# Themaister/Granite

Hardware: NVIDIA H100
Metric: frames/sec (higher is better)
Workload: dtype f32

## Files before the change

granite_b200/csrc/grb_post.cu:

```cuda
#include "grb_common.cuh"

#include <cooperative_groups.h>

#include <algorithm>
#include <cstdio>
#include <cstdlib>

namespace grb
{
namespace
{
constexpr int kBlockX = 32;
constexpr int kBlockY = 8;

inline dim3 grid_for(int w, int rows) { return dim3((w + kBlockX - 1) / kBlockX, (rows + kBlockY - 1) / kBlockY, 1); }

template <bool DynamicExposure, typename HdrTexel = uint32_t>
__global__ void __launch_bounds__(kBlockX *kBlockY) bloom_threshold_kernel(View<const HdrTexel> hdr, const float *__restrict__ lum,
                                                                          View<uint2> out, int y0, int y1, float inv_w, float inv_h)
{
	int x = blockIdx.x * kBlockX + threadIdx.x;
	int y = y0 + blockIdx.y * kBlockY + threadIdx.y;
	if (x >= out.w || y >= y1)
		return;
// ... 420 lines not shown
	float3 a0 = sample_unorm8(in, u + dx * k0, v + dy * k0);
	float3 a1 = sample_unorm8(in, u + dx * k1, v + dy * k1);
	float3 rgbA = make_float3(0.5f * (a0.x + a1.x), 0.5f * (a0.y + a1.y), 0.5f * (a0.z + a1.z));
	float3 b0 = sample_unorm8(in, u + dx * -0.5f, v + dy * -0.5f);
	float3 b1 = sample_unorm8(in, u + dx * 0.5f, v + dy * 0.5f);
	float3 rgbB = make_float3(rgbA.x * 0.5f + 0.25f * (b0.x + b1.x), rgbA.y * 0.5f + 0.25f * (b0.y + b1.y), rgbA.z * 0.5f + 0.25f * (b0.z + b1.z));
	float lumaB = luma_of(rgbB);
	float3 c = ((lumaB < lumaMin) || (lumaB > lumaMax)) ? rgbA : rgbB;
	uint32_t px;
	if (SrgbTarget)
		px = linear_to_srgb8(decode_srgb1(c.x)) | (linear_to_srgb8(decode_srgb1(c.y)) << 8) | (linear_to_srgb8(decode_srgb1(c.z)) << 16);
	else
		px = float_to_unorm8(c.x) | (float_to_unorm8(c.y) << 8) | (float_to_unorm8(c.z) << 16);
	out.at(x, y) = px | 0xff000000u;
#undef fetch_unorm8
#undef sample_unorm8
}

__device__ __forceinline__ float3 hdr_to_taa(float3 c)
{
	c = make_float3(c.x * 8.0f, c.y * 8.0f, c.z * 8.0f);
	float r = 1.0f / (fmax_(c.x, fmax_(c.y, c.z)) + 1.0f);
	c = make_float3(c.x * r, c.y * r, c.z * r);
	return make_float3(0.25f * c.x + 0.5f * c.y + 0.25f * c.z, 0.5f * c.y - 0.25f * c.x - 0.25f * c.z, 0.5f * c.x - 0.5f * c.z);
}

__device__ __forceinline__ float3 taa_to_hdr(float3 c)
{
	float tmp = c.x - c.y;
	float3 rgb = make_float3(fclamp(tmp + c.z, 0.0f, 0.999f), fclamp(c.x + c.y, 0.0f, 0.999f), fclamp(tmp - c.z, 0.0f, 0.999f));
	float r = 1.0f / (1.0f - fmax_(rgb.x, fmax_(rgb.y, rgb.z)));
	return make_float3((1.0f / 8.0f) * rgb.x * r, (1.0f / 8.0f) * rgb.y * r, (1.0f / 8.0f) * rgb.z * r);
}

__device__ __forceinline__ float3 min3(float3 a, float3 b) { return make_float3(fmin_(a.x, b.x), fmin_(a.y, b.y), fmin_(a.z, b.z)); }
__device__ __forceinline__ float3 max3(float3 a, float3 b) { return make_float3(fmax_(a.x, b.x), fmax_(a.y, b.y), fmax_(a.z, b.z)); }

template <bool Aabb>
__device__ __forceinline__ float3 clamp_box(float3 color, float3 lo, float3 hi)
{
	if (!Aabb)
		return make_float3(fclamp(color.x, lo.x, hi.x), fclamp(color.y, lo.y, hi.y), fclamp(color.z, lo.z, hi.z));
	float3 center = make_float3(0.5f * (lo.x + hi.x), 0.5f * (lo.y + hi.y), 0.5f * (lo.z + hi.z));
	float3 radius = make_float3(fmax_(0.5f * (hi.x - lo.x), 0.0001f), fmax_(0.5f * (hi.y - lo.y), 0.0001f), fmax_(0.5f * (hi.z - lo.z), 0.0001f));
	float3 v = make_float3(color.x - center.x, color.y - center.y, color.z - center.z);
	float3 units = make_float3(v.x / radius.x, v.y / radius.y, v.z / radius.z);
	float max_unit = fmax_(fmax_(fabsf(units.x), fabsf(units.y)), fabsf(units.z));
	if (max_unit > 1.0f)
		return make_float3(center.x + v.x / max_unit, center.y + v.y / max_unit, center.z + v.z / max_unit);
	return color;
}

template <typename HdrTexel>
struct TaaInputsT
{
	View<const HdrTexel> hdr;
	View<const float> depth;
	View<const uint32_t> mv;
	View<const uint2> history;
};
using TaaInputs = TaaInputsT<uint32_t>;

__device__ __forceinline__ float3 sample_rgb16f(const View<const uint2> &im, float u, float v)
{
	float4 s = sample_rgba16f(im, u, v);
	return make_float3(s.x, s.y, s.z);
}

__device__ __forceinline__ float3 sample_catmull_rom(const View<const uint2> &tex, float u, float v, float4 rt)
{
	float spx = u * rt.z, spy = v * rt.w;
	float t1x = floorf(spx - 0.5f) + 0.5f, t1y = floorf(spy - 0.5f) + 0.5f;
	float fx = spx - t1x, fy = spy - t1y;
#define GRB_W0(f) ((f) * (-0.5f + (f) * (1.0f - 0.5f * (f))))
#define GRB_W1(f) (1.0f + (f) * (f) * (-2.5f + 1.5f * (f)))
#define GRB_W2(f) ((f) * (0.5f + (f) * (2.0f - 1.5f * (f))))
#define GRB_W3(f) ((f) * (f) * (-0.5f + 0.5f * (f)))
	float w0x = GRB_W0(fx), w1x = GRB_W1(fx), w2x = GRB_W2(fx), w3x = GRB_W3(fx);
	float w0y = GRB_W0(fy), w1y = GRB_W1(fy), w2y = GRB_W2(fy), w3y = GRB_W3(fy);
#undef GRB_W0
#undef GRB_W1
#undef GRB_W2
#undef GRB_W3
	float w12x = w1x + w2x, w12y = w1y + w2y;
	float o12x = w2x / (w1x + w2x), o12y = w2y / (w1y + w2y);
	float t0x = (t1x - 1.0f) * rt.x, t0y = (t1y - 1.0f) * rt.y;
	float t3x = (t1x + 2.0f) * rt.x, t3y = (t1y + 2.0f) * rt.y;
	float t12x = (t1x + o12x) * rt.x, t12y = (t1y + o12y) * rt.y;
	float3 result = make_float3(0.0f, 0.0f, 0.0f);
#define GRB_ACC(UU, VV, WA, WB)                      \
	{                                                \
		float4 s4 = sample_rgba16f_snap(tex, (UU), (VV)); float3 s = make_float3(s4.x, s4.y, s4.z); \
		result.x += s.x * (WA) * (WB);               \
		result.y += s.y * (WA) * (WB);               \
		result.z += s.z * (WA) * (WB);               \
	}
	GRB_ACC(t0x, t0y, w0x, w0y)
	GRB_ACC(t12x, t0y, w12x, w0y)
	GRB_ACC(t3x, t0y, w3x, w0y)
	GRB_ACC(t0x, t12y, w0x, w12y)
	GRB_ACC(t12x, t12y, w12x, w12y)
	GRB_ACC(t3x, t12y, w3x, w12y)
	GRB_ACC(t0x, t3y, w0x, w3y)
	GRB_ACC(t12x, t3y, w12x, w3y)
	GRB_ACC(t3x, t3y, w3x, w3y)
#undef GRB_ACC
	return result;
}

struct Mat4
{
	float m[16];
};

template <int Quality, bool History, typename HdrTexel = uint32_t>
__global__ void __launch_bounds__(kBlockX *kBlockY) taa_kernel(TaaInputsT<HdrTexel> in, Mat4 reproj, View<uint32_t> out_color, View<uint2> out_history, int y0,
                                                              int y1, float4 rt)
{
	int x = blockIdx.x * kBlockX + threadIdx.x;
	int y = y0 + blockIdx.y * kBlockY + threadIdx.y;
	if (x >= out_color.w || y >= y1)
		return;
	const int w = in.hdr.w, h = in.hdr.h;
#define GRB_CUR(DX, DY) hdr_to_taa(fetch_hdr_clamped(in.hdr, x + (DX), y + (DY)))
	float3 current = GRB_CUR(0, 0);
	float3 out_c = current;
	if (History)
	{
		float u = ((float)x + 0.5f) * rt.x, v = ((float)y + 0.5f) * rt.y;
		float d;
		uint32_t mvp;
#define GRB_TRY(PX, PY)                                                 \
	{                                                                   \
		int qx = iclamp((PX), 0, w - 1), qy = iclamp((PY), 0, h - 1);   \
		float dd = __ldg(&in.depth.at(qx, qy));                         \
		if (dd > d)                                                     \
		{                                                               \
			d = dd;                                                     \
			mvp = __ldg(&in.mv.at(qx, qy));                             \
		}                                                               \
	}
		if (Quality == 2)
		{
			int qx = iclamp(x + 1, 0, w - 1), qy = iclamp(y + 1, 0, h - 1);
			d = __ldg(&in.depth.at(qx, qy));
			mvp = __ldg(&in.mv.at(qx, qy));
			GRB_TRY(x - 1, y) GRB_TRY(x, y) GRB_TRY(x, y - 1) GRB_TRY(x - 1, y - 1)
			GRB_TRY(x + 1, y) GRB_TRY(x + 1, y - 1)
			GRB_TRY(x - 1, y + 1) GRB_TRY(x, y + 1)
		}
		else
		{
			int qx = iclamp(x - 1, 0, w - 1);
			d = __ldg(&in.depth.at(qx, y));
			mvp = __ldg(&in.mv.at(qx, y));
			GRB_TRY(x, y) GRB_TRY(x, y - 1) GRB_TRY(x, y + 1) GRB_TRY(x + 1, y)
		}
#undef GRB_TRY
		float mvx = h2f((uint16_t)(mvp & 0xffffu)), mvy = h2f((uint16_t)(mvp >> 16));
		float old_u, old_v;
		if (mvx == 0.0f && mvy == 0.0f)
		{
			float cx = 2.0f * u - 1.0f, cy = 2.0f * v - 1.0f;
			const float *m = reproj.m;
			float px = m[0] * cx + m[4] * cy + m[8] * d + m[12] * 1.0f;
			float py = m[1] * cx + m[5] * cy + m[9] * d + m[13] * 1.0f;
			float pw = m[3] * cx + m[7] * cy + m[11] * d + m[15] * 1.0f;
			old_u = px / pw;
			old_v = py / pw;
			mvx = u - old_u;
			mvy = v - old_v;
		}
		else
		{
			old_u = u - mvx;
			old_v = v - mvy;
		}
		float3 hist = Quality == 2 ? sample_catmull_rom(in.history, old_u, old_v, rt) : sample_rgb16f(in.history, old_u, old_v);
		float mv_len = sqrtf(mvx * mvx + mvy * mvy);
		float mv_fast = fmin_(mv_len * 50.0f, 1.0f);
		float gamma = fmix(1.5f, 0.5f, mv_fast);
		hist = make_float3(fclamp(hist.x, 0.0f, 1.0f), fclamp(hist.y, -1.0f, 1.0f), fclamp(hist.z, -1.0f, 1.0f));
		float lerp_factor = (1.0f + 2.0f * mv_fast) / 16.0f;

		float3 c11 = current;
		float3 c01 = GRB_CUR(-1, 0), c21 = GRB_CUR(+1, 0), c10 = GRB_CUR(0, -1), c12 = GRB_CUR(0, +1);
		float3 lo = c11, hi = c11;
		if (Quality == 0 || Quality == 1)
		{
			lo = min3(lo, c01); lo = min3(lo, c21); lo = min3(lo, c10); lo = min3(lo, c12);
			hi = max3(hi, c01); hi = max3(hi, c21); hi = max3(hi, c10); hi = max3(hi, c12);
		}
		if (Quality >= 1)
		{
			float3 corner_lo = lo, corner_hi = hi;
			float3 c00 = GRB_CUR(-1, -1), c22 = GRB_CUR(+1, +1), c02 = GRB_CUR(-1, +1), c20 = GRB_CUR(+1, -1);
			if (Quality == 1)
			{
				lo = min3(lo, c00); lo = min3(lo, c22); lo = min3(lo, c02); lo = min3(lo, c20);
				hi = max3(hi, c00); hi = max3(hi, c22); hi = max3(hi, c02); hi = max3(hi, c20);
				lo = make_float3(0.5f * (corner_lo.x + lo.x), 0.5f * (corner_lo.y + lo.y), 0.5f * (corner_lo.z + lo.z));
				hi = make_float3(0.5f * (corner_hi.x + hi.x), 0.5f * (corner_hi.y + hi.y), 0.5f * (corner_hi.z + hi.z));
			}
			else
			{
#define GRB_M1(C) ((c00.C + 2.0f * c01.C + c02.C + 2.0f * c10.C + 4.0f * c11.C + 2.0f * c12.C + c20.C + 2.0f * c21.C + c22.C) / 16.0f)
#define GRB_M2(C)                                                                                                                            \
	(c00.C * c00.C + 2.0f * c01.C * c01.C + c02.C * c02.C + 2.0f * c10.C * c10.C + 4.0f * c11.C * c11.C + 2.0f * c12.C * c12.C + c20.C * c20.C + \
	 2.0f * c21.C * c21.C + c22.C * c22.C)
				float3 m1 = make_float3(GRB_M1(x), GRB_M1(y), GRB_M1(z));
				float3 m2 = make_float3(GRB_M2(x), GRB_M2(y), GRB_M2(z));
#undef GRB_M1
#undef GRB_M2
				float3 sigma = make_float3(sqrtf(fmax_(m2.x / 16.0f - m1.x * m1.x, 0.0f)), sqrtf(fmax_(m2.y / 16.0f - m1.y * m1.y, 0.0f)),
				                           sqrtf(fmax_(m2.z / 16.0f - m1.z * m1.z, 0.0f)));
				lo = make_float3(m1.x - gamma * sigma.x, m1.y - gamma * sigma.y, m1.z - gamma * sigma.z);
				hi = make_float3(m1.x + gamma * sigma.x, m1.y + gamma * sigma.y, m1.z + gamma * sigma.z);
			}
		}
		hist = clamp_box<Quality != 0>(hist, lo, hi);
		out_c = make_float3(fmix(hist.x, current.x, lerp_factor), fmix(hist.y, current.y, lerp_factor), fmix(hist.z, current.z, lerp_factor));
	}
#undef GRB_CUR
	float3 color = taa_to_hdr(out_c);
	out_color.at(x, y) = pack_r11g11b10(color.x, color.y, color.z);
	out_history.at(x, y) = pack_rgba16f(make_float4(out_c.x, out_c.y, out_c.z, 1.0f));
}

__device__ __forceinline__ float4 sample_rgba16f_cg(const View<const uint2> &im, float u, float v)
{
	Bilin s = bilin_setup(u, v, im.w, im.h);
	float4 t00 = unpack_rgba16f(__ldcg(&im.at(s.x0, s.y0)));
	float4 t10 = unpack_rgba16f(__ldcg(&im.at(s.x1, s.y0)));
	float4 t01 = unpack_rgba16f(__ldcg(&im.at(s.x0, s.y1)));
	float4 t11 = unpack_rgba16f(__ldcg(&im.at(s.x1, s.y1)));
	return bilin_mix4(t00, t10, t01, t11, s.a, s.b);
}

__device__ __forceinline__ float4 tent9_cg(const View<const uint2> &src, float u, float v, float off, float inv_in_w, float inv_in_h)
{
	const float du = off * inv_in_w, dv = off * inv_in_h;
	const float um = u + (-du), up = u + du;
	const float vm = v + (-dv), vp = v + dv;
	float4 s = sample_rgba16f_cg(src, u, v);
	float4 acc = make_float4(0.25f * s.x, 0.25f * s.y, 0.25f * s.z, 0.25f * s.w);
#define GRB_TAP(W, U, V)                     \
	s = sample_rgba16f_cg(src, (U), (V));    \
	acc.x += (W)*s.x;                        \
	acc.y += (W)*s.y;                        \
	acc.z += (W)*s.z;                        \
	acc.w += (W)*s.w;
	GRB_TAP(0.0625f, um, vp)
	GRB_TAP(0.125f, u, vp)
	GRB_TAP(0.0625f, up, vp)
	GRB_TAP(0.125f, um, v)
	GRB_TAP(0.125f, up, v)
	GRB_TAP(0.0625f, um, vm)
	GRB_TAP(0.125f, u, vm)
	GRB_TAP(0.0625f, up, vm)
#undef GRB_TAP
	return acc;
}

struct TailArgs
{
	View<const uint2> d0;
	View<uint2> d1, d2, d3, u2, u1;
	View<const uint2> history;
	float lerp_d3;
	float *lum;
	float lerp_lum, lo, hi;
	View<uint2> u0;
	int u0_y0, u0_y1;
	const uint32_t *wait_flags;
	int wait_count;
	uint32_t wait_epoch;
	uint32_t *error_word;
	unsigned max_spins;
};

constexpr int kTailThreads = 1024;

__device__ __forceinline__ void tail_level(const View<const uint2> &src, const View<uint2> &dst, float off, const View<const uint2> *history, float lerp,
                                          unsigned first_cta, unsigned num_ctas, int y0 = 0, int y1 = -1)
{
	const float inv_w = 1.0f / (float)dst.w, inv_h = 1.0f / (float)dst.h, inv_in_w = 1.0f / (float)src.w, inv_in_h = 1.0f / (float)src.h;
	if (y1 < 0)
		y1 = dst.h;
	const int total = dst.w * (y1 - y0);
	for (int i = (int)((blockIdx.x - first_cta) * kTailThreads + threadIdx.x); i < total; i += (int)(num_ctas * kTailThreads))
	{
		const int yr = i / dst.w, x = i - yr * dst.w, y = y0 + yr;
		const float u = ((float)x + 0.5f) * inv_w, v = ((float)y + 0.5f) * inv_h;
		float4 value = tent9_cg(src, u, v, off, inv_in_w, inv_in_h);
		if (history)
		{
			const float4 hs = unpack_rgba16f(__ldg(&history->at(x, y)));
			value = make_float4(fmix(hs.x, value.x, lerp), fmix(hs.y, value.y, lerp), fmix(hs.z, value.z, lerp), fmix(hs.w, value.w, 1.0f));
		}
		dst.at(x, y) = pack_rgba16f(value);
	}
}

__global__ void __launch_bounds__(kTailThreads) bloom_tail_kernel(const TailArgs a)
{
	namespace cg = cooperative_groups;
	cg::grid_group grid = cg::this_grid();
	__shared__ float s_grid[kLumFastMaxSamples];
	__shared__ float s_part[64];
	auto as_src = [](const View<uint2> &v) { return View<const uint2>{ v.p, v.w, v.h, v.pitch }; };
	if (a.wait_flags)
	{
		if ((int)threadIdx.x < a.wait_count)
			for (unsigned spins = 0; (int32_t)(load_acquire_system(a.wait_flags + threadIdx.x) - a.wait_epoch) < 0; spins++)
			{
				if (spins > a.max_spins)
				{
					if (blockIdx.x == 0)
						printf("granite_b200: timed out waiting for rank %d's band of frame %u\n", (int)threadIdx.x, a.wait_epoch);
					if (a.error_word)
					{
						*reinterpret_cast<volatile uint32_t *>(a.error_word) = (GRB_DEVICE_ERROR_PEER_TIMEOUT << 24) | ((uint32_t)threadIdx.x << 16) | (a.wait_epoch & 0xffffu);
						__threadfence_system();
					}
					break;
				}
				__nanosleep(128);
			}
		__syncthreads();
	}
	tail_level(a.d0, a.d1, 1.75f, nullptr, 0.0f, 0u, gridDim.x);
	grid.sync();
	tail_level(as_src(a.d1), a.d2, 1.75f, nullptr, 0.0f, 0u, gridDim.x);
	grid.sync();
	tail_level(as_src(a.d2), a.d3, 1.75f, a.history.p ? &a.history : nullptr, a.lerp_d3, 0u, gridDim.x);
	grid.sync();
	const bool lum_cta = a.lum != nullptr && blockIdx.x == 0 && gridDim.x > 1;
	if (a.lum != nullptr && (lum_cta || gridDim.x == 1))
	{
		const View<const uint2> d3 = as_src(a.d3);
		const int size_x = d3.w / 2, size_y = d3.h / 2;
		const float inv_sx = 1.0f / (float)size_x, inv_sy = 1.0f / (float)size_y;
		for (int i = threadIdx.x; i < size_x * size_y; i += kTailThreads)
		{
			const int sy = i / size_x, sx = i - sy * size_x;
			s_grid[i] = sample_rgba16f_cg(d3, ((float)sx + 0.5f) * inv_sx, ((float)sy + 0.5f) * inv_sy).w;
		}
		__syncthreads();
		if (threadIdx.x < 64)
		{
			const int iter_y = (size_y + 7) >> 3, iter_x = (size_x + 7) >> 3;
			const int lx = threadIdx.x & 7, ly = threadIdx.x >> 3;
			float total = 0.0f;
			for (int y = 0; y < iter_y; y++)
				for (int x = 0; x < iter_x; x++)
				{
					const int sx = x * 8 + lx, sy = y * 8 + ly;
					if (sx < size_x && sy < size_y)
						total += s_grid[sy * size_x + sx];
				}
			s_part[threadIdx.x] = total;
		}
		luminance_tail(s_part, threadIdx.x, size_x, size_y, inv_sx, inv_sy, a.lum, a.lerp_lum, a.lo, a.hi);
	}
	if (!lum_cta)
		tail_level(as_src(a.d3), a.u2, 0.875f, nullptr, 0.0f, a.lum != nullptr && gridDim.x > 1 ? 1u : 0u, a.lum != nullptr && gridDim.x > 1 ? gridDim.x - 1u : gridDim.x);
	grid.sync();
	tail_level(as_src(a.u2), a.u1, 0.875f, nullptr, 0.0f, 0u, gridDim.x);
	if (a.u0.p)
	{
		grid.sync();
		tail_level(as_src(a.u1), a.u0, 0.875f, nullptr, 0.0f, 0u, gridDim.x, a.u0_y0, a.u0_y1);
	}
}
}
}

namespace grb
{
bool launch_tent_tiled(bool up, const GrbImage *in, const GrbImage *history, float lerp, const GrbImage *out, GrbRows rows, cudaStream_t stream, int32_t *rc);
bool launch_tonemap_fast(const GrbImage *hdr, const GrbImage *bloom, const float *luminance, float exposure, const GrbImage *out, GrbRows rows, cudaStream_t stream,
                         int32_t *rc);
bool launch_fxaa_fast(const GrbImage *in, const GrbImage *out, GrbRows rows, cudaStream_t stream, int32_t *rc);
bool launch_taa_fast(const GrbImage *hdr, const GrbImage *depth, const GrbImage *mv, const GrbImage *history, const float *reproj16, const GrbImage *out_color,
                     const GrbImage *out_history, GrbRows rows, cudaStream_t stream, int32_t *rc);
}

using namespace grb;

extern "C" int32_t grb_bloom_threshold(const GrbImage *hdr, const float *luminance, const GrbImage *out, GrbRows rows, void *stream)
{
	const bool hdr16 = image_ok(hdr, GRB_FORMAT_R16G16B16A16_SFLOAT, 8);
	if ((!hdr16 && !image_ok(hdr, GRB_FORMAT_B10G11R11_UFLOAT_PACK32, 4)) || !image_ok(out, GRB_FORMAT_R16G16B16A16_SFLOAT, 8))
	{
		set_last_error("grb_bloom_threshold: hdr must be B10G11R11_UFLOAT or R16G16B16A16_SFLOAT and out R16G16B16A16_SFLOAT");
		return GRB_ERR_UNSUPPORTED_FORMAT;
	}
	rows = full_rows(rows, out->height);
	if (rows.y1 <= rows.y0)
		return GRB_OK;
	auto o = view_of<uint2>(out);
	dim3 grid = grid_for(out->width, rows.y1 - rows.y0), block(kBlockX, kBlockY);
	float inv_w = 1.0f / (float)out->width, inv_h = 1.0f / (float)out->height;
	if (hdr16)
	{
		if (luminance)
			bloom_threshold_kernel<true, uint2><<<grid, block, 0, as_stream(stream)>>>(view_of<const uint2>(hdr), luminance, o, rows.y0, rows.y1, inv_w, inv_h);
		else
			bloom_threshold_kernel<false, uint2><<<grid, block, 0, as_stream(stream)>>>(view_of<const uint2>(hdr), nullptr, o, rows.y0, rows.y1, inv_w, inv_h);
		return check_launch("grb_bloom_threshold");
	}
	if (luminance)
		bloom_threshold_kernel<true><<<grid, block, 0, as_stream(stream)>>>(view_of<const uint32_t>(hdr), luminance, o, rows.y0, rows.y1, inv_w, inv_h);
	else
		bloom_threshold_kernel<false><<<grid, block, 0, as_stream(stream)>>>(view_of<const uint32_t>(hdr), nullptr, o, rows.y0, rows.y1, inv_w, inv_h);
	return check_launch("grb_bloom_threshold");
}

extern "C" int32_t grb_bloom_downsample(const GrbImage *in, const GrbImage *history, float lerp, const GrbImage *out, GrbRows rows, void *stream)
{
	if (!image_ok(in, GRB_FORMAT_R16G16B16A16_SFLOAT, 8) || !image_ok(out, GRB_FORMAT_R16G16B16A16_SFLOAT, 8) ||
	    (history && (!image_ok(history, GRB_FORMAT_R16G16B16A16_SFLOAT, 8) || history->width != out->width || history->height != out->height)))
	{
		set_last_error("grb_bloom_downsample: images must be R16G16B16A16_SFLOAT and history must match out");
		return GRB_ERR_UNSUPPORTED_FORMAT;
	}
	if (history && history->data == out->data)
	{
		set_last_error("grb_bloom_downsample: history must not alias the output");
		return GRB_ERR_INVALID_ARGUMENT;
	}
	rows = full_rows(rows, out->height);
	if (rows.y1 <= rows.y0)
		return GRB_OK;
	{
		int32_t rc = GRB_OK;
		if (launch_tent_tiled(false, in, history, lerp, out, rows, as_stream(stream), &rc))
			return rc;
	}
	dim3 grid = grid_for(out->width, rows.y1 - rows.y0), block(kBlockX, kBlockY);
	float inv_w = 1.0f / (float)out->width, inv_h = 1.0f / (float)out->height;
	float inv_in_w = 1.0f / (float)in->width, inv_in_h = 1.0f / (float)in->height;
	if (history)
		bloom_downsample_kernel<true><<<grid, block, 0, as_stream(stream)>>>(view_of<const uint2>(in), view_of<const uint2>(history), lerp,
		                                                                      view_of<uint2>(out), rows.y0, rows.y1, inv_w, inv_h, inv_in_w, inv_in_h);
	else
		bloom_downsample_kernel<false><<<grid, block, 0, as_stream(stream)>>>(view_of<const uint2>(in), View<const uint2>{}, lerp, view_of<uint2>(out),
		                                                                       rows.y0, rows.y1, inv_w, inv_h, inv_in_w, inv_in_h);
	return check_launch("grb_bloom_downsample");
}

extern "C" int32_t grb_bloom_downsample_to_peers(const GrbImage *in, const GrbImage *out_layout, void *const *peer_images, uint32_t *const *peer_flags,
                                                 int32_t peer_count, int32_t flag_index, uint32_t epoch, uint32_t *scratch_counter, GrbRows rows,
                                                 void *stream)
{
	if (!image_ok(in, GRB_FORMAT_R16G16B16A16_SFLOAT, 8) || !out_layout || out_layout->format != GRB_FORMAT_R16G16B16A16_SFLOAT || !peer_images ||
	    !peer_flags || !scratch_counter || peer_count < 1 || peer_count > GRB_MAX_PEERS || flag_index < 0 || (out_layout->row_pitch % 8) != 0)
	{
		set_last_error("grb_bloom_downsample_to_peers: bad arguments");
		return GRB_ERR_INVALID_ARGUMENT;
	}
	rows = full_rows(rows, out_layout->height);
	PeerTargets targets{};
	targets.count = peer_count;
	for (int r = 0; r < peer_count; r++)
	{
		if (!peer_images[r] || !peer_flags[r])
		{
			set_last_error("grb_bloom_downsample_to_peers: null peer pointer");
			return GRB_ERR_INVALID_ARGUMENT;
		}
		targets.data[r] = static_cast<uint2 *>(peer_images[r]);
		targets.flags[r] = peer_flags[r];
	}
	const int row_count = rows.y1 > rows.y0 ? rows.y1 - rows.y0 : 0;
	dim3 grid = grid_for(out_layout->width, row_count > 0 ? row_count : 1), block(kBlockX, kBlockY);
	if (row_count == 0)
		grid = dim3(1, 1, 1);
	bloom_downsample_peers_kernel<<<grid, block, 0, as_stream(stream)>>>(
	    view_of<const uint2>(in), targets, row_count > 0 ? out_layout->width : 0, out_layout->row_pitch / 8, rows.y0, rows.y0 + row_count,
	    1.0f / (float)out_layout->width, 1.0f / (float)out_layout->height, 1.0f / (float)in->width, 1.0f / (float)in->height, flag_index, epoch,
	    scratch_counter);
	return check_launch("grb_bloom_downsample_to_peers");
}

extern "C" int32_t grb_peer_wait(const uint32_t *local_flags, int32_t count, uint32_t epoch, void *stream)
{
	if (!local_flags || count < 1 || count > GRB_MAX_PEERS)
	{
		set_last_error("grb_peer_wait: bad arguments");
		return GRB_ERR_INVALID_ARGUMENT;
	}
	unsigned max_spins = 1u << 25;
	if (const char *e = getenv("GRB_PEER_WAIT_SPINS"))
		max_spins = (unsigned)strtoul(e, nullptr, 10);
	peer_wait_kernel<<<1, 32, 0, as_stream(stream)>>>(local_flags, count, epoch, device_error_word(), max_spins);
	return check_launch("grb_peer_wait");
}

static int32_t bloom_upsample_impl(const GrbImage *in, const GrbImage *out, GrbRows rows, void *stream, bool allow_tiles)
{
	if (!image_ok(in, GRB_FORMAT_R16G16B16A16_SFLOAT, 8) || !image_ok(out, GRB_FORMAT_R16G16B16A16_SFLOAT, 8))
	{
		set_last_error("grb_bloom_upsample: images must be R16G16B16A16_SFLOAT");
		return GRB_ERR_UNSUPPORTED_FORMAT;
	}
	rows = full_rows(rows, out->height);
	if (rows.y1 <= rows.y0)
		return GRB_OK;
	if (allow_tiles)
	{
		int32_t rc = GRB_OK;
		if (launch_tent_tiled(true, in, nullptr, 0.0f, out, rows, as_stream(stream), &rc))
			return rc;
	}
	dim3 grid = grid_for(out->width, rows.y1 - rows.y0), block(kBlockX, kBlockY);
	bloom_upsample_kernel<<<grid, block, 0, as_stream(stream)>>>(view_of<const uint2>(in), view_of<uint2>(out), rows.y0, rows.y1,
	                                                              1.0f / (float)out->width, 1.0f / (float)out->height, 1.0f / (float)in->width,
	                                                              1.0f / (float)in->height);
	return check_launch("grb_bloom_upsample");
}

extern "C" int32_t grb_bloom_upsample(const GrbImage *in, const GrbImage *out, GrbRows rows, void *stream)
{
	return bloom_upsample_impl(in, out, rows, stream, true);
}

extern "C" int32_t grb_bloom_upsample_exact(const GrbImage *in, const GrbImage *out, GrbRows rows, void *stream)
{
	return bloom_upsample_impl(in, out, rows, stream, false);
}

extern "C" int32_t grb_luminance(const GrbImage *d3, float *luminance, float lerp, float min_loglum, float max_loglum, void *stream)
{
	if (!image_ok(d3, GRB_FORMAT_R16G16B16A16_SFLOAT, 8) || !luminance || d3->width < 2 || d3->height < 2)
	{
		set_last_error("grb_luminance: d3 must be R16G16B16A16_SFLOAT (>= 2x2) and luminance non-null");
		return GRB_ERR_INVALID_ARGUMENT;
	}
	if ((d3->width / 2) * (d3->height / 2) <= kLumFastMaxSamples)
		luminance_fast_kernel<<<1, kLumFastThreads, 0, as_stream(stream)>>>(view_of<const uint2>(d3), luminance, lerp, min_loglum, max_loglum);
	else
		luminance_kernel<<<1, 64, 0, as_stream(stream)>>>(view_of<const uint2>(d3), luminance, lerp, min_loglum, max_loglum);
	return check_launch("grb_luminance");
}

extern "C" int32_t grb_luminance_grid(const GrbImage *d3, float *grid, GrbRows rows, void *stream)
{
	if (!image_ok(d3, GRB_FORMAT_R16G16B16A16_SFLOAT, 8) || !grid || d3->width < 2 || d3->height < 2)
	{
		set_last_error("grb_luminance_grid: d3 must be R16G16B16A16_SFLOAT (>= 2x2) and grid non-null");
		return GRB_ERR_INVALID_ARGUMENT;
	}
	rows = full_rows(rows, d3->height / 2);
	if (rows.y1 <= rows.y0)
		return GRB_OK;
	dim3 grid_dim = grid_for(d3->width / 2, rows.y1 - rows.y0), block(kBlockX, kBlockY);
	luminance_grid_kernel<<<grid_dim, block, 0, as_stream(stream)>>>(view_of<const uint2>(d3), grid, rows.y0, rows.y1);
	return check_launch("grb_luminance_grid");
}

extern "C" int32_t grb_luminance_finalize(const float *grid, int32_t size_x, int32_t size_y, float *luminance, float lerp, float min_loglum,
                                          float max_loglum, void *stream)
{
	if (!grid || !luminance || size_x <= 0 || size_y <= 0)
	{
		set_last_error("grb_luminance_finalize: null grid/luminance or empty size");
		return GRB_ERR_INVALID_ARGUMENT;
	}
	luminance_finalize_kernel<<<1, 64, 0, as_stream(stream)>>>(grid, size_x, size_y, luminance, lerp, min_loglum, max_loglum);
	return check_launch("grb_luminance_finalize");
}

extern "C" int32_t grb_tonemap(const GrbImage *hdr, const GrbImage *bloom, const float *luminance, float dynamic_exposure, const GrbImage *out,
                               GrbRows rows, void *stream)
{
	bool srgb = out && out->format == GRB_FORMAT_R8G8B8A8_SRGB;
	const bool hdr16 = image_ok(hdr, GRB_FORMAT_R16G16B16A16_SFLOAT, 8);
	if ((!hdr16 && !image_ok(hdr, GRB_FORMAT_B10G11R11_UFLOAT_PACK32, 4)) || !image_ok(bloom, GRB_FORMAT_R16G16B16A16_SFLOAT, 8) ||
	    !(image_ok(out, GRB_FORMAT_R8G8B8A8_SRGB, 4) || image_ok(out, GRB_FORMAT_R8G8B8A8_UNORM, 4)) || out->width != hdr->width ||
	    out->height != hdr->height)
	{
		set_last_error("grb_tonemap: hdr B10G11R11_UFLOAT or R16G16B16A16_SFLOAT, bloom R16G16B16A16_SFLOAT, out R8G8B8A8_{SRGB,UNORM} of hdr's size");
		return GRB_ERR_UNSUPPORTED_FORMAT;
	}
	rows = full_rows(rows, out->height);
	if (rows.y1 <= rows.y0)
		return GRB_OK;
	dim3 grid = grid_for(out->width, rows.y1 - rows.y0), block(kBlockX, kBlockY);
	float inv_w = 1.0f / (float)out->width, inv_h = 1.0f / (float)out->height;
	auto b = view_of<const uint2>(bloom);
	auto o = view_of<uint32_t>(out);
	cudaStream_t s = as_stream(stream);
	if (hdr16)
	{
		auto h16 = view_of<const uint2>(hdr);
		if (luminance && srgb)
			tonemap_kernel<true, true, uint2><<<grid, block, 0, s>>>(h16, b, luminance, dynamic_exposure, o, rows.y0, rows.y1, inv_w, inv_h);
		else if (luminance)
			tonemap_kernel<true, false, uint2><<<grid, block, 0, s>>>(h16, b, luminance, dynamic_exposure, o, rows.y0, rows.y1, inv_w, inv_h);
		else if (srgb)
			tonemap_kernel<false, true, uint2><<<grid, block, 0, s>>>(h16, b, nullptr, dynamic_exposure, o, rows.y0, rows.y1, inv_w, inv_h);
		else
			tonemap_kernel<false, false, uint2><<<grid, block, 0, s>>>(h16, b, nullptr, dynamic_exposure, o, rows.y0, rows.y1, inv_w, inv_h);
		return check_launch("grb_tonemap");
	}
	auto h = view_of<const uint32_t>(hdr);
	{
		int32_t rc = GRB_OK;
		if (launch_tonemap_fast(hdr, bloom, luminance, dynamic_exposure, out, rows, s, &rc))
			return rc;
	}
	const bool vec4 = (out->width % 4) == 0 && bloom->width * 4 == out->width && (hdr->row_pitch % 16) == 0 && (out->row_pitch % 16) == 0 &&
	                  (reinterpret_cast<uintptr_t>(hdr->data) % 16) == 0 && (reinterpret_cast<uintptr_t>(out->data) % 16) == 0;
	if (vec4)
	{
		dim3 grid4((out->width / 4 + kBlockX - 1) / kBlockX, (rows.y1 - rows.y0 + kBlockY - 1) / kBlockY, 1);
		if (luminance && srgb)
			tonemap4_kernel<true, true><<<grid4, block, 0, s>>>(h, b, luminance, dynamic_exposure, o, rows.y0, rows.y1, inv_w, inv_h);
		else if (luminance)
			tonemap4_kernel<true, false><<<grid4, block, 0, s>>>(h, b, luminance, dynamic_exposure, o, rows.y0, rows.y1, inv_w, inv_h);
		else if (srgb)
			tonemap4_kernel<false, true><<<grid4, block, 0, s>>>(h, b, nullptr, dynamic_exposure, o, rows.y0, rows.y1, inv_w, inv_h);
		else
			tonemap4_kernel<false, false><<<grid4, block, 0, s>>>(h, b, nullptr, dynamic_exposure, o, rows.y0, rows.y1, inv_w, inv_h);
		return check_launch("grb_tonemap");
	}
	if (luminance && srgb)
		tonemap_kernel<true, true><<<grid, block, 0, s>>>(h, b, luminance, dynamic_exposure, o, rows.y0, rows.y1, inv_w, inv_h);
	else if (luminance)
		tonemap_kernel<true, false><<<grid, block, 0, s>>>(h, b, luminance, dynamic_exposure, o, rows.y0, rows.y1, inv_w, inv_h);
	else if (srgb)
		tonemap_kernel<false, true><<<grid, block, 0, s>>>(h, b, nullptr, dynamic_exposure, o, rows.y0, rows.y1, inv_w, inv_h);
	else
		tonemap_kernel<false, false><<<grid, block, 0, s>>>(h, b, nullptr, dynamic_exposure, o, rows.y0, rows.y1, inv_w, inv_h);
	return check_launch("grb_tonemap");
}

extern "C" int32_t grb_fxaa(const GrbImage *in, const GrbImage *out, GrbRows rows, void *stream)
{
	auto is8 = [](const GrbImage *im) { return image_ok(im, GRB_FORMAT_R8G8B8A8_SRGB, 4) || image_ok(im, GRB_FORMAT_R8G8B8A8_UNORM, 4); };
	if (!is8(in) || !is8(out) || in->width != out->width || in->height != out->height || in->data == out->data)
	{
		set_last_error("grb_fxaa: in/out must be distinct R8G8B8A8 images of equal size");
		return GRB_ERR_UNSUPPORTED_FORMAT;
	}
	rows = full_rows(rows, out->height);
	if (rows.y1 <= rows.y0)
		return GRB_OK;
	{
		int32_t rc = GRB_OK;
		if (launch_fxaa_fast(in, out, rows, as_stream(stream), &rc))
			return rc;
	}
	dim3 grid = grid_for(out->width, rows.y1 - rows.y0), block(kBlockX, kBlockY);
	float inv_w = 1.0f / (float)in->width, inv_h = 1.0f / (float)in->height;
	if (out->format == GRB_FORMAT_R8G8B8A8_SRGB)
		fxaa_kernel<true><<<grid, block, 0, as_stream(stream)>>>(view_of<const uint32_t>(in), view_of<uint32_t>(out), rows.y0, rows.y1, inv_w, inv_h);
	else
		fxaa_kernel<false><<<grid, block, 0, as_stream(stream)>>>(view_of<const uint32_t>(in), view_of<uint32_t>(out), rows.y0, rows.y1, inv_w, inv_h);
	return check_launch("grb_fxaa");
}

extern "C" int32_t grb_taa_resolve(const GrbImage *hdr, const GrbImage *depth, const GrbImage *mv, const GrbImage *history, const float *reproj16,
                                   int32_t quality, const GrbImage *out_color, const GrbImage *out_history, GrbRows rows, void *stream)
{
	const bool hdr16 = image_ok(hdr, GRB_FORMAT_R16G16B16A16_SFLOAT, 8);
	if ((!hdr16 && !image_ok(hdr, GRB_FORMAT_B10G11R11_UFLOAT_PACK32, 4)) || !image_ok(out_color, GRB_FORMAT_B10G11R11_UFLOAT_PACK32, 4) ||
	    !image_ok(out_history, GRB_FORMAT_R16G16B16A16_SFLOAT, 8) || out_color->width != hdr->width || out_color->height != hdr->height ||
	    out_history->width != hdr->width || out_history->height != hdr->height)
	{
		set_last_error("grb_taa_resolve: hdr B10G11R11_UFLOAT or R16G16B16A16_SFLOAT, out_color B10G11R11_UFLOAT, out_history R16G16B16A16_SFLOAT, equal sizes");
		return GRB_ERR_UNSUPPORTED_FORMAT;
	}
	if (history && (!image_ok(history, GRB_FORMAT_R16G16B16A16_SFLOAT, 8) || !image_ok(depth, GRB_FORMAT_D32_SFLOAT, 4) ||
// ... 186 lines not shown
```

Baseline: 1871.

## Stage separable horizontal lerps in shared memory for bloom tail upsample

Replaces the per-pixel 9-tap tent upsample in the cooperative bloom tail kernel with a tiled version. Each CTA first computes horizontal bilinear lerps for the needed source rows into a shared buffer, then each thread finishes the vertical blend from shared memory. This cuts redundant global texel loads and interpolation work across neighbouring pixels. The cost is a 32KB shared buffer (also reused for the luminance grid), extra __syncthreads per tile, and a fallback path when a tile's rows do not fit.

Measured after the change: 1951 (median of 6 runs). 4.3% higher.

```diff
diff --git a/granite_b200/csrc/grb_post.cu b/granite_b200/csrc/grb_post.cu
--- a/granite_b200/csrc/grb_post.cu
+++ b/granite_b200/csrc/grb_post.cu
@@ -746,11 +746,88 @@
 	}
 }
 
+constexpr int kUpTile = 32;
+constexpr int kUpLerpSlots = 2048;
+static_assert(kUpTile * kUpTile == kTailThreads, "one texel per thread");
+
+__device__ __forceinline__ void tail_upsample_level(const View<const uint2> &src, const View<uint2> &dst, float4 *lerps, unsigned first_cta,
+                                                   unsigned num_ctas, int y0 = 0, int y1 = -1)
+{
+	const float off = 0.875f;
+	const float inv_w = 1.0f / (float)dst.w, inv_h = 1.0f / (float)dst.h, inv_in_w = 1.0f / (float)src.w, inv_in_h = 1.0f / (float)src.h;
+	const float du = fmul(off, inv_in_w), dv = fmul(off, inv_in_h);
+	if (y1 < 0)
+		y1 = dst.h;
+	const int tiles_x = (dst.w + kUpTile - 1) / kUpTile, tiles = tiles_x * ((y1 - y0 + kUpTile - 1) / kUpTile);
+	const int c = (int)threadIdx.x & (kUpTile - 1), ry = (int)threadIdx.x / kUpTile;
+	for (int tile = (int)(blockIdx.x - first_cta); tile < tiles; tile += (int)num_ctas)
+	{
+		const int tx0 = (tile % tiles_x) * kUpTile, ty0 = y0 + (tile / tiles_x) * kUpTile, ty_last = min(ty0 + kUpTile, y1) - 1;
+		const float v_first = ((float)ty0 + 0.5f) * inv_h, v_last = ((float)ty_last + 0.5f) * inv_h;
+		const int r_lo = bilin_setup(0.5f, fadd(v_first, -dv), src.w, src.h).y0, r_hi = bilin_setup(0.5f, fadd(v_last, dv), src.w, src.h).y1;
+		const int n_rows = r_hi - r_lo + 1;
+		const int x = tx0 + c, y = ty0 + ry;
+		const bool mine = x < dst.w && y <= ty_last;
+		const float u = ((float)x + 0.5f) * inv_w, v = ((float)y + 0.5f) * inv_h;
+		if (n_rows * 3 * kUpTile > kUpLerpSlots)
+		{
+			if (mine)
+				dst.at(x, y) = pack_rgba16f(tent9_cg(src, u, v, off, inv_in_w, inv_in_h));
+			continue;
+		}
+		__syncthreads();
+		for (int j = (int)threadIdx.x; j < n_rows * 3 * kUpTile; j += kTailThreads)
+		{
+			const int col = j & (kUpTile - 1), t = (j / kUpTile) % 3, r = r_lo + j / (3 * kUpTile);
+			const float uc = ((float)(tx0 + col) + 0.5f) * inv_w;
+			const float ut = t == 0 ? fadd(uc, -du) : (t == 1 ? uc : fadd(uc, du));
+			const Bilin s = bilin_setup(ut, 0.5f, src.w, src.h);
+			const float4 t0 = unpack_rgba16f(__ldcg(&src.at(s.x0, r))), t1 = unpack_rgba16f(__ldcg(&src.at(s.x1, r)));
+			const float ia = fsub(1.0f, s.a);
+			lerps[j] = make_float4(fadd(fmul(t0.x, ia), fmul(t1.x, s.a)), fadd(fmul(t0.y, ia), fmul(t1.y, s.a)), fadd(fmul(t0.z, ia), fmul(t1.z, s.a)),
+			                       fadd(fmul(t0.w, ia), fmul(t1.w, s.a)));
+		}
+		__syncthreads();
+		if (!mine)
+			continue;
+		const float vt[3] = { fadd(v, -dv), v, fadd(v, dv) };
+		int row0[3], row1[3];
+		float wb[3], wib[3];
+#pragma unroll
+		for (int k = 0; k < 3; k++)
+		{
+			const Bilin s = bilin_setup(u, vt[k], src.w, src.h);
+			row0[k] = (s.y0 - r_lo) * 3 * kUpTile + c;
+			row1[k] = (s.y1 - r_lo) * 3 * kUpTile + c;
+			wb[k] = s.b;
+			wib[k] = fsub(1.0f, s.b);
+		}
+		const auto tap = [&](int t, int k) {
+			const float4 top = lerps[row0[k] + t * kUpTile], bot = lerps[row1[k] + t * kUpTile];
+			return make_float4(fadd(fmul(top.x, wib[k]), fmul(bot.x, wb[k])), fadd(fmul(top.y, wib[k]), fmul(bot.y, wb[k])),
+			                   fadd(fmul(top.z, wib[k]), fmul(bot.z, wb[k])), fadd(fmul(top.w, wib[k]), fmul(bot.w, wb[k])));
+		};
+		float4 s0 = tap(1, 1);
+		float4 acc = make_float4(fmul(0.25f, s0.x), fmul(0.25f, s0.y), fmul(0.25f, s0.z), fmul(0.25f, s0.w));
+		const int tt[8] = { 0, 1, 2, 0, 2, 0, 1, 2 }, tk[8] = { 2, 2, 2, 1, 1, 0, 0, 0 };
+		const float wt[8] = { 0.0625f, 0.125f, 0.0625f, 0.125f, 0.125f, 0.0625f, 0.125f, 0.0625f };
+#pragma unroll
+		for (int i = 0; i < 8; i++)
+		{
+			s0 = tap(tt[i], tk[i]);
+			acc = make_float4(fadd(acc.x, fmul(wt[i], s0.x)), fadd(acc.y, fmul(wt[i], s0.y)), fadd(acc.z, fmul(wt[i], s0.z)), fadd(acc.w, fmul(wt[i], s0.w)));
+		}
+		dst.at(x, y) = pack_rgba16f(acc);
+	}
+}
+
 __global__ void __launch_bounds__(kTailThreads) bloom_tail_kernel(const TailArgs a)
 {
 	namespace cg = cooperative_groups;
 	cg::grid_group grid = cg::this_grid();
-	__shared__ float s_grid[kLumFastMaxSamples];
+	__shared__ float4 s_lerps[kUpLerpSlots];
+	static_assert(kUpLerpSlots * 4 >= kLumFastMaxSamples, "the luminance grid shares the buffer");
+	float *const s_grid = reinterpret_cast<float *>(s_lerps);
 	__shared__ float s_part[64];
 	auto as_src = [](const View<uint2> &v) { return View<const uint2>{ v.p, v.w, v.h, v.pitch }; };
 	if (a.wait_flags)
@@ -808,13 +885,13 @@
 		luminance_tail(s_part, threadIdx.x, size_x, size_y, inv_sx, inv_sy, a.lum, a.lerp_lum, a.lo, a.hi);
 	}
 	if (!lum_cta)
-		tail_level(as_src(a.d3), a.u2, 0.875f, nullptr, 0.0f, a.lum != nullptr && gridDim.x > 1 ? 1u : 0u, a.lum != nullptr && gridDim.x > 1 ? gridDim.x - 1u : gridDim.x);
+		tail_upsample_level(as_src(a.d3), a.u2, s_lerps, a.lum != nullptr && gridDim.x > 1 ? 1u : 0u, a.lum != nullptr && gridDim.x > 1 ? gridDim.x - 1u : gridDim.x);
 	grid.sync();
-	tail_level(as_src(a.u2), a.u1, 0.875f, nullptr, 0.0f, 0u, gridDim.x);
+	tail_upsample_level(as_src(a.u2), a.u1, s_lerps, 0u, gridDim.x);
 	if (a.u0.p)
 	{
 		grid.sync();
-		tail_level(as_src(a.u1), a.u0, 0.875f, nullptr, 0.0f, 0u, gridDim.x, a.u0_y0, a.u0_y1);
+		tail_upsample_level(as_src(a.u1), a.u0, s_lerps, 0u, gridDim.x, a.u0_y0, a.u0_y1);
 	}
 }
 }
```
